# gynvael/MythTracer

Measured on AMD Instinct MI355X. Metric: Mray/s (primary+shadow+secondary; ray = one OctTree::IntersectRay), higher is better.
Workload: dtype f64

## Files before the change

### include/mythtracer_hip.h

```cpp
#ifndef MYTHTRACER_HIP_H_
#define MYTHTRACER_HIP_H_

#include <stdint.h>

#ifdef __cplusplus
extern "C" {
#endif

#define MT_ABI_VERSION 5

enum {
  MT_OK = 0,
  MT_ERR_ARG = -1,
  MT_ERR_HIP = -2,
  MT_ERR_UNSUPPORTED = -3,
  MT_ERR_NOMEM = -4,
  MT_ERR_INTERNAL = -5
};

#define MT_MAX_TREE_DEPTH 64
#define MT_MAX_RECURSION 16

typedef struct mt_material {
  double ambient[3], diffuse[3], specular[3];
// ... 301 lines not shown
  MT_TUNE_HYBRID_QUAD_SHARE,
  MT_TUNE_HYBRID_WORK1, MT_TUNE_HYBRID_WORK2,
  MT_TUNE_FORECAST_STEP,
  MT_TUNE_HYBRID_STARTER_SHARE,
  MT_TUNE_DEEP_LAYOUT,
  MT_TUNE_MULTI_FORCE_PEER_COPY,
  MT_TUNE_MULTI_BALANCE,
  MT_TUNE_XCD_QUEUES,
  MT_TUNE_ORDER_GROUPS,
  MT_TUNE_SM_CELL_SHARE,
  MT_TUNE_SM_CELL_TIME, MT_TUNE_SM_CELL_WORK,
  MT_TUNE_HYBRID_CELL_FACTOR,
  MT_TUNE_LEAN_KERNEL,
  MT_TUNE_COUNT
};
int mt_scene_set_tuning(mt_scene *scene, int knob, double value);

int mt_scene_kernel_times(mt_scene *scene, int max_n, double *primary_ms,
                          double *render_ms);

typedef struct mt_lean_info {
  int32_t lean, handed_over;
  uint32_t units, redo_units;
  double lean_ms, redo_ms;
} mt_lean_info;
int mt_scene_lean_info(mt_scene *scene, mt_lean_info *out);

int mt_intersect_rays(mt_scene *scene, int n, const double *rays,
                      int32_t *tri, int32_t *line_no, double *t,
                      double *point, mt_stats *stats);
// ... 58 lines not shown
```

### mythtracer_amd/binding.py

```python
from __future__ import annotations

import ctypes as C
import os
import weakref

import numpy as np

PKG = os.path.dirname(os.path.abspath(__file__))
HIP_LIB = os.path.join(PKG, "lib", "libmythtracer_hip.so")
HOST_LIB = os.path.join(PKG, "lib", "libmythtracer_host.so")

MT_OK = 0
MT_ABI_VERSION = 5
MT_TEX_RGB8, MT_TEX_F64 = 0, 1

HIP_SYMBOLS = [
    "mt_last_error", "mt_abi_version", "mt_device_count", "mt_scene_create",
    "mt_scene_destroy", "mt_scene_set_lights", "mt_render_chunk",
    "mt_render_chunk_device", "mt_render_tiles_device", "mt_blit_tiles_device",
    "mt_scene_read_stats", "mt_intersect_rays", "mt_scene_set_traversal_mode",
    "mt_scene_kernel_times", "mt_scene_lean_info", "mt_scene_set_scheduling", "mt_scene_set_engine",
    "mt_scene_set_stats", "mt_set_default_engine", "mt_scene_set_tuning",
    "mt_render_frame_multi", "mt_scene_export_costs_device", "mt_scene_import_costs_device",
    "mt_order_tiles_device", "mt_dealt_tile_count", "mt_deal_tiles_device",
# ... 17 lines not shown
    "mt_scene_set_triangle_normals", "mt_scene_set_triangle_uvw", "mt_scene_get_triangle_normals",
    "mt_scene_get_triangle_uvw", "mt_raytree_attr_info_last",
    "mt_octree_build", "mt_octree_info", "mt_octree_read", "mt_octree_destroy", "mt_scene_create_triangles",
    "mt_scene_read_tree",
    "mt_scene_set_triangle_vertices", "mt_scene_get_triangle_vertices", "mt_scene_move_times_last",
]
MT_MAX_RECURSION = 16

TUNE = {name: i for i, name in enumerate([
    "POOL_BELOW", "POOL_CAP", "PACKED_STACK", "BLOCKS_PER_CU", "FORECAST_RADIUS", "BLEND", "FORMS",
    "POOL_CUT_SHARE", "POOL_PIECE_TIME1", "POOL_PIECE_TIME2", "POOL_PIECE_WORK1", "POOL_PIECE_WORK2",
    "POOL_CELL_FACTOR", "QUAD_SHARE", "QUAD_SHARE_MOVING", "QUAD_KEEP", "QUAD_WORK", "QUAD_WORK_MOVING",
    "POOL_SCRATCH_MB", "HYBRID_POOL_SHARE", "HYBRID_QUAD_SHARE", "HYBRID_WORK1", "HYBRID_WORK2", "FORECAST_STEP",
    "HYBRID_STARTER_SHARE", "DEEP_LAYOUT", "MULTI_FORCE_PEER_COPY", "MULTI_BALANCE", "XCD_QUEUES",
    "ORDER_GROUPS", "SM_CELL_SHARE", "SM_CELL_TIME", "SM_CELL_WORK", "HYBRID_CELL_FACTOR", "LEAN_KERNEL"])}

STAT_NAMES = ["rays_primary", "rays_secondary", "rays_shadow", "box_tests",
              "node_visits", "tri_tests", "mt_tests", "shaded_hits"]


class NativeLibraryMissing(RuntimeError):
    pass


class mt_material(C.Structure):
    _fields_ = [("ambient", C.c_double * 3), ("diffuse", C.c_double * 3),
                ("specular", C.c_double * 3), ("specular_exp", C.c_double),
                ("reflectance", C.c_double), ("transparency", C.c_double),
                ("transmission_filter", C.c_double * 3),
                ("refraction_index", C.c_double), ("tex", C.c_int32),
# ... 991 lines not shown
    def read_stats(self, h) -> dict:
        st = mt_stats()
        self.check(self.lib.mt_scene_read_stats(h, C.byref(st)))
        return st.as_dict()

    def set_stats(self, h, enabled: bool):
        self.check(self.lib.mt_scene_set_stats(h, 1 if enabled else 0))

    def set_engine(self, h, engine: int):
        self.check(self.lib.mt_scene_set_engine(h, int(engine)))

    def set_default_engine(self, engine: int):
        self.check(self.lib.mt_set_default_engine(int(engine)))

    def set_tuning(self, h, knob: str, value: float):
        self.check(self.lib.mt_scene_set_tuning(h, TUNE[knob], float(value)))

    def render_frame_multi(self, handles, sensor12, image_w, image_h, tile_w=64, tile_h=64, max_depth=5,
                           want_stats=True):
        n = len(handles)
        arr = (C.c_void_p * n)(*handles)
        rgb = np.zeros((image_h, image_w, 3), dtype=np.uint8)
        st = (mt_stats * n)()
        s = self.make_sensor(sensor12)
        self.check(self.lib.mt_render_frame_multi(C.cast(arr, C.c_void_p), n, C.byref(s), image_w, image_h,
                                                  tile_w, tile_h, max_depth, _ptr(rgb),
                                                  C.cast(st, C.c_void_p) if want_stats else None))
        return dict(rgb=rgb, stats=[st[i].as_dict() for i in range(n)])

    def export_costs_device(self, h, d_map, map_w, map_h, stream=None):
        self.check(self.lib.mt_scene_export_costs_device(h, d_map, map_w, map_h, stream))
# ... 635 lines not shown
```

### mythtracer_amd/csrc/mt_capi.hip

```cpp
#include <hip/hip_runtime.h>
#include <algorithm>
#include <atomic>
#include <map>
#include <memory>
#include <mutex>
#include <string>
#include <thread>
#include <limits>
#include <utility>

#include <chrono>
#include <cmath>
#include <cstdarg>
#include <cstddef>
#include <cstdio>
#include <cstdlib>
#include <cstring>
#include <unistd.h>
#include <vector>

#include "mt_render.hip"
#include "mt_resolve.h"
#include "mt_adaptive.h"
#include "mt_gbuffer.h"
// ... 196 lines not shown
struct mt_scene {
  int device = 0;
  DevScene dev{};
  DeviceAllocs geo, tables;
  TriArrays tri;
  mt_material *mtls = nullptr;
  DevTexture *texs = nullptr;
  Buf<mt_light> d_lights;
  Buf<unsigned long long> d_counters;
  Buf<unsigned int> d_work;
  Buf<unsigned int> d_queues;
  Buf<unsigned int> d_order_ctl;
  Buf<unsigned int> d_order_whist;
  unsigned order_epoch = 0;
  DevScene dev_uploaded;
  bool dev_uploaded_valid = false;
  Buf<double> d_frames;
  Buf<int32_t> d_hit_prim;
  Buf<double> d_hit_t;
  Buf<unsigned int> d_class_list;
  Buf<char> d_pool;
  int engine = 0;
  ForecastBank bank0;
  std::unique_ptr<ForecastBank> bank1;
  void forget_histories() {
    bank0.cost_signature = 0;
    if (bank1) bank1->cost_signature = 0;
    lean_fresh = true;
  }
  bool lean_fresh = true;
// ... 833 lines not shown
  MT_TRY(geo.upload(L.supers, "the super boxes", &dev->sup_aabb32));
  MT_TRY(geo.upload(L.subs, "the subtree boxes", &dev->sub_aabb32));
  MT_TRY(geo.upload(L.hsr, "the walk's records", &dev->hs_rec));
  MT_TRY(geo.upload(L.ll_tri, "the long lists", &dev->ll_tri));
  MT_TRY(geo.upload(L.ll_exact, "the long lists", &dev->ll_exact));
  MT_TRY(geo.upload(L.ll_box_q, "the long lists' boxes", &dev->ll_box_q));
  MT_TRY(geo.upload(L.ll_grp_q, "the long lists' boxes", &dev->ll_grp_q));
  MT_TRY(geo.upload(L.ll_sup_q, "the long lists' boxes", &dev->ll_sup_q));
  MT_TRY(geo.upload(L.sl_box, "the short lists' boxes", &dev->sl_box32));
  MT_TRY(geo.upload(L.recs, "the node records", &dev->nodes));
  MT_TRY(geo.upload(L.tri_aabb, "the triangles' boxes", &dev->tri_aabb));
  MT_TRY(geo.upload(L.tri_aabb32, "the triangles' boxes", &dev->tri_aabb32));
  for (int k = 0; k < 3; k++) dev->bmax[k] = L.bmax[k];
  dev->tree_depth = L.max_depth;
  dev->scene_regular = L.regular ? 1 : 0;
  return MT_OK;
}

static void show_tri_arrays(const TriArrays &tri, DevScene *dev) {
  dev->tri_vertex = tri.vertex;
  dev->tri_normal = tri.normal;
  dev->tri_uvw = tri.uvw;
  dev->tri_mtl = tri.mtl;
  dev->tri_line = tri.line;
}

static int upload_layout(mt_scene *s, const mt_scene_desc *d, const SceneLayout &L) {
  HIP_TRY(hipSetDevice(d->device));
  s->device = d->device;
  hipDeviceProp_t prop;
// ... 23 lines not shown
    texs[i] = DevTexture{dev_texels, t.width, t.height, t.format, 0};
  }
  MT_TRY(s->tables.upload(d->materials, (size_t)d->n_materials, "the materials", &s->mtls));
  s->dev.mtls = s->mtls;
  s->n_materials = d->n_materials;
  s->n_textures = d->n_textures;
  if (d->n_materials > 0) s->mtls_host.assign(d->materials, d->materials + d->n_materials);
  MT_TRY(s->tables.upload(texs, "the texture table", &s->texs));
  s->dev.texs = s->texs;
  s->texs_host = texs;
  s->tex_generation.assign(texs.size(), 0ull);
  s->dev.n_tris = d->n_tris;
  s->dev.n_nodes = d->n_nodes;
  s->dev.force_mode = 0;
  s->dev.pack_shift = pack_shift_for(d->n_tris, d->n_nodes);
  s->dev.n_lights = 0;
  s->dev.lights = nullptr;
  return MT_OK;
}

static int init_launch_state(mt_scene *s) {
  MT_TRY(s->d_counters.ensure(ST_COUNT * sizeof(unsigned long long)));
  HIP_TRY(hipMemset(s->d_counters, 0, ST_COUNT * sizeof(unsigned long long)));
  MT_TRY(s->d_work.ensure((kLeanCtl + 8) * sizeof(unsigned)));
  HIP_TRY(hipMemset(s->d_work, 0, (kLeanCtl + 8) * sizeof(unsigned)));
  MT_TRY(s->d_queues.ensure(kQueueWords * sizeof(unsigned)));
  MT_TRY(s->d_order_ctl.ensure(kOrdWords * sizeof(unsigned)));
  HIP_TRY(hipMemset(s->d_order_ctl, 0, kOrdWords * sizeof(unsigned)));
  MT_TRY(s->d_order_whist.ensure((size_t)kOrdGroupsMax * kOrdKeysMax * sizeof(unsigned)));
  HIP_TRY(hipEventCreate(&s->ev0));
// ... 280 lines not shown

int mt_scene_set_engine(mt_scene *s, int engine) {
  if (!s || engine < 0 || engine > 3) return fail(MT_ERR_ARG, "engine must be 0 (automatic), 1, 2 or 3");
  s->engine = engine;
  s->forget_histories();
  return MT_OK;
}

int mt_set_default_engine(int engine) {
  if (engine < 0 || engine > 3) return fail(MT_ERR_ARG, "engine must be 0 (automatic), 1, 2 or 3");
  g_default_engine.store(engine);
  return MT_OK;
}

int mt_scene_set_tuning(mt_scene *s, int knob, double value) {
  if (!s || knob < 0 || knob >= MT_TUNE_COUNT || !std::isfinite(value)) return fail(MT_ERR_ARG, "bad tuning argument");
  switch (knob) {
    case MT_TUNE_POOL_PIECE_TIME1: case MT_TUNE_POOL_PIECE_TIME2: case MT_TUNE_POOL_PIECE_WORK1: case MT_TUNE_POOL_PIECE_WORK2:
    case MT_TUNE_POOL_CELL_FACTOR: case MT_TUNE_QUAD_SHARE: case MT_TUNE_QUAD_SHARE_MOVING: case MT_TUNE_QUAD_KEEP:
    case MT_TUNE_QUAD_WORK: case MT_TUNE_QUAD_WORK_MOVING: case MT_TUNE_HYBRID_POOL_SHARE: case MT_TUNE_HYBRID_QUAD_SHARE:
    case MT_TUNE_SM_CELL_SHARE: case MT_TUNE_SM_CELL_TIME: case MT_TUNE_SM_CELL_WORK: case MT_TUNE_HYBRID_CELL_FACTOR:
    case MT_TUNE_HYBRID_WORK1: case MT_TUNE_HYBRID_WORK2: case MT_TUNE_FORECAST_STEP: case MT_TUNE_HYBRID_STARTER_SHARE:
      if (!(value >= 1e-6 && value <= 1e6)) return fail(MT_ERR_ARG, "tuning knob %d must lie in [1e-6, 1e6]", knob);
      break;
    case MT_TUNE_POOL_BELOW: case MT_TUNE_POOL_CAP: case MT_TUNE_BLOCKS_PER_CU:
      if (!(value >= 0.0 && value <= 1e9)) return fail(MT_ERR_ARG, "tuning knob %d must lie in [0, 1e9]", knob);
      break;
    case MT_TUNE_POOL_SCRATCH_MB:
      if (!(value >= 1.0 && value <= 1e9)) return fail(MT_ERR_ARG, "the ray pool's scratch budget must lie in [1, 1e9] MB");
      break;
// ... 2937 lines not shown
```

### mythtracer_amd/csrc/mt_device.h

```cpp
#pragma once
#include <hip/hip_runtime.h>
#include <stddef.h>
#include <stdint.h>
#include "mythtracer_hip.h"

#ifndef MT_WAVES_PER_SIMD
#define MT_WAVES_PER_SIMD 2
#endif

namespace mt {

struct NodeRec {
  double lo[3];
  double c[3];
  double hi[3];
  int32_t first_child;
  int32_t prim_begin;
  int32_t prim_count;
  int32_t child_mask;
  int32_t level;
  int32_t pad1;
};
static_assert(sizeof(NodeRec) == 96, "NodeRec must be 96 bytes");

// ... 59 lines not shown
  const double *tri_vertex;
  const double *tri_normal;
  const double *tri_uvw;
  const int32_t *tri_mtl;
  const int32_t *tri_line;
  const mt_material *mtls;
  const DevTexture *texs;
  const mt_light *lights;
  int32_t n_lights;
  int32_t n_tris;
  int32_t n_nodes;
  int32_t tree_depth;
  int32_t force_mode;
  int32_t scene_regular;
  int32_t pack_shift;
  volatile unsigned long long *hb;
  unsigned long long *prof;
  char *deep_base;
  unsigned long long deep_stride;
  const DevScene *self;
};

constexpr int kProfTimeline = 16384;
enum { PROF_TRACE = 0, PROF_SCAN_RAYPAR, PROF_SCAN_TRANSPOSED, PROF_CHILDREN_UNWIND, PROF_N_RAYPAR,
       PROF_N_TRANSPOSED, PROF_N_CHUNKS, PROF_N_RAYPAR_TRIS, PROF_N_TRACES, PROF_SHADE,
       PROF_SCAN_M2F, PROF_SCAN_M2, PROF_SCAN_M1, PROF_SCAN_M0, PROF_N_M2F, PROF_N_M2, PROF_N_M1, PROF_N_M0,
       PROF_TRIS_M2F, PROF_TRIS_M1, PROF_TRIS_TRANSPOSED,
       PROF_G_GROUPS, PROF_G_LIVE, PROF_G_RANGES, PROF_G_RANGE_TRIS,
       PROF_NIN_SUM, PROF_NIN_LT8, PROF_NIN_LT24, PROF_WANT_SUM,
       PROF_TA_G, PROF_TB_G, PROF_TA_T, PROF_TB_T, PROF_TC_T, PROF_T_RAYS, PROF_M2F_CALL,
// ... 122 lines not shown
```

### mythtracer_amd/csrc/mt_layout.h

```cpp
#pragma once
#include <algorithm>
#include <cmath>
#include <cstdarg>
#include <cstddef>
#include <cstdio>
#include <cstring>
#include <string>
#include <utility>
#include <vector>

#include "mt_device.h"

namespace mt {

struct LayoutError {
  int code = MT_OK;
  std::string msg;
};

inline bool refuse(LayoutError *err, int code, const char *fmt, ...) {
  char text[1024];
  va_list ap;
  va_start(ap, fmt);
  vsnprintf(text, sizeof text, fmt, ap);
  va_end(ap);
  err->code = code;
// ... 79 lines not shown

struct SceneLayout {
  std::vector<NodeRec> recs;
  std::vector<float> groups;
  std::vector<float> supers;
  std::vector<float> subs;
  std::vector<HsRec> hsr;
  std::vector<float> sl_box;
  std::vector<int32_t> ll_tri;
  std::vector<double> ll_exact;
  std::vector<float> ll_box_q, ll_grp_q, ll_sup_q;
  std::vector<double> tri_aabb;
  std::vector<float> tri_aabb32;
  double bmax[3] = {0.0, 0.0, 0.0};
  bool regular = false;
  int max_depth = 0;
};


constexpr double kInvertedBox[6] = {3.0e38, 3.0e38, 3.0e38, -3.0e38, -3.0e38, -3.0e38};
static_assert((float)3.0e38 == 3.0e38f, "the fp32 inverted box is the rounded fp64 one");

template <typename T>
inline void box_invert(T *u) {
  for (int k = 0; k < 6; k++) u[k] = (T)kInvertedBox[k];
}

template <typename T>
inline void box_union(T *u, const T *b, size_t n = 1) {
  for (size_t j = 0; j < n; j++, b += 6) {
// ... 253 lines not shown
}

inline void derive_layout(const mt_scene_desc &d, const std::vector<int> &depth_of, SceneLayout *out) {
  SceneLayout &L = *out;
  L = SceneLayout();
  L.regular = scene_regular(d);
  L.max_depth = *std::max_element(depth_of.begin(), depth_of.end());
  derive_node_records(d, depth_of, &L.recs);
  derive_block_boxes(d, &L.groups, &L.supers);
  derive_subtree_boxes(d, &L.recs, &L.subs);
  derive_hit_set_records(d, L.recs, L.subs, &L.hsr, &L.sl_box);
  std::vector<float> ll_box;
  derive_long_lists(d, &L.hsr, &L.ll_tri, &L.ll_exact, &ll_box);
  derive_long_list_quads(ll_box, &L);
  derive_triangle_boxes(d, &L);
}

}
```

### mythtracer_amd/csrc/mt_render.hip

```cpp
#include "mt_shade.h"
#include "mt_pool.h"

namespace mt {

enum { MODE_RADIANCE = 0, MODE_SHADOW = 1 };
enum { STAGE_REFL = 0, STAGE_REFR = 1 };

constexpr int kParkSlots = 18;
enum { PARK_START = 0, PARK_LP = 3, PARK_ADD1 = 6, PARK_ADD2 = 9, PARK_ADD3 = 12, PARK_DIR = 15 };
struct FrameIO {
  double *base;
  double *park;
  int lane;
  __device__ __forceinline__ void park3(int s, V3 v) const {
    park[(s + 0) * 64 + lane] = v.x; park[(s + 1) * 64 + lane] = v.y; park[(s + 2) * 64 + lane] = v.z;
  }
  __device__ __forceinline__ V3 unpark3(int s) const {
    return V3{park[(s + 0) * 64 + lane], park[(s + 1) * 64 + lane], park[(s + 2) * 64 + lane]};
  }
  __device__ __forceinline__ double *slot(int level, int s) const {
    return base + ((size_t)level * kFrameSlots + s) * 64 + lane;
  }
  __device__ __forceinline__ void put3(int level, int s, V3 v) const {
    *slot(level, s) = v.x; *slot(level, s + 1) = v.y; *slot(level, s + 2) = v.z;
// ... 330 lines not shown
    }

    const unsigned long long item_t0 = __builtin_amdgcn_s_memtime();
#ifdef MT_DIAG
    unsigned long long diag_trace_ticks = 0;
#endif
    const ItemGeom g = item_geometry<!LEAN>(P, item, sub, lane);
    bool alive = g.inside;
    const size_t px_index = g.px_index;

    const bool quad = sub >= 0;
    const int R = quad ? 4 : 1;
    const int role = quad ? (lane & 3) : 0;
    const bool owner = role == 0;
    const unsigned long long my_group = quad ? (0xFull << (lane & ~3)) : (1ull << lane);
    enum { MODE_IDLE = 2 };
    int mode = owner ? MODE_RADIANCE : MODE_IDLE;
    int level = 0;
    bool in_object = false;
    double coef = 1.0;
    V3 ro = cam_origin, rd = v3(0, 0, 1);
    if (alive) {
      const V3 d = s_start + (s_ds * (double)g.py) + (s_dp * (double)g.px);
      rd = normalized(d);
    }
    V3 Pt = v3(0, 0, 0), Nn = Pt, surf = Pt, color = Pt;
    bool has_light = false, has_add3 = false, crossed = false;
    double refl_dot = 0.0;
    int mtl = -1, li = 0, round_base = 0;
    bool traversing = false;
    bool want_round = false, waiting_round = false;

    const long long pass_bound =
        (2ll << P.max_depth) * (1 + (long long)S.n_lights * ((long long)S.n_tris + 2)) + 16;
    long long passes = 0;
    while (__ballot(alive) != 0ull) {
      int prim = -1;
      double t = 0.0;
      if (heartbeat) {
        const unsigned long long am = __ballot(alive);
        const unsigned long long ex = __builtin_amdgcn_read_exec();
        if (lane == 0) {
          S.hb[wave_id * 4 + 0] = 2 | ((unsigned long long)passes << 8);
          S.hb[wave_id * 4 + 2] = am;
          S.hb[wave_id * 4 + 3] = ex;
        }
      }
      int trc = DEV_OK;
      const bool tracing = alive && mode != MODE_IDLE;
      if (passes == 0 && from_primary) {
        prim = tracing ? P.hit_prim[px_index] : -1;
        t = tracing ? P.hit_t[px_index] : 0.0;
      } else {
#ifdef MT_DIAG
        const unsigned long long diag_tt0 = __builtin_amdgcn_s_memtime();
#endif
        const TraceOut to = trace_wave<STATS, DEEP, LEAN>(S.self, stk.base, lane, tracing, ro.x, ro.y, ro.z, rd.x, rd.y, rd.z);
#ifdef MT_DIAG
        asm volatile("" :: "v"(to.prim));
        diag_trace_ticks += __builtin_amdgcn_s_memtime() - diag_tt0;
#endif
        add_trace_stats<STATS>(st, to);
        prim = to.prim;
        t = to.t;
        trc = to.status;
        if (LEAN && __builtin_amdgcn_readfirstlane(trc) == DEV_NEEDS_FULL) {
          abandon = true;
          break;
        }
      }
      if (heartbeat) {
        const unsigned long long ex = __builtin_amdgcn_read_exec();
        if (lane == 0) { S.hb[wave_id * 4 + 0] = 3 | ((unsigned long long)passes << 8); S.hb[wave_id * 4 + 3] = ex; }
      }
      if (trc != DEV_OK || ++passes > pass_bound) {
        if (lane == 0) atomicMax(P.counters + ST_STATUS, (unsigned long long)(trc != DEV_OK ? trc : DEV_ERR_PIXEL_BOUND));
        alive = false;
        break;
      }

      bool after_lights = false, do_return = false;
      V3 retval = v3(0, 0, 0);
      V3 add1 = retval, add2 = retval, add3 = retval;
      if (tracing) {
        if (mode == MODE_RADIANCE) {
          if (STATS) {
            if (level > 0) st.v[ST_RAYS_SECONDARY]++;
            else if (!from_primary) st.v[ST_RAYS_PRIMARY]++;
          }
          if (prim < 0) {
            do_return = true;
          } else {
            if (STATS) {
              st.v[ST_SHADED_HITS]++;
              st.v[ST_BYTES_VECTOR] += 72u + 72u + 4u + 64u;
            }
            Pt = ro + rd * t;
            const V3 dir = rd;
            const double *vtx = S.tri_vertex + (size_t)prim * 9;
// ... 16 lines not shown
              if (m->tex >= 0) {
                const V3 uvw = interpolate(S.tri_uvw + (size_t)prim * 9, w);
                surf = surf * texture_color_at(S.texs[m->tex], uvw.x, uvw.y);
              }
              const V3 Rd = dir - Nn * (2 * dot(dir, Nn));
              refl_dot = dot(Rd, towards_camera);
              fio.park3(PARK_DIR, dir);
              color = v3(0, 0, 0);
              round_base = 0;
              if (S.n_lights > 0) want_round = true;
              else after_lights = true;
              mode = MODE_IDLE;
            }
          }
        } else {
          if (STATS) {
            st.v[ST_RAYS_SHADOW]++;
            st.v[ST_BYTES_VECTOR] += 96u + 4u + 32u;
          }
          const MT_CONST mt_light *lt = lights + li;
          const V3 lpos = v3(lt->position[0], lt->position[1], lt->position[2]);
          bool light_done = false, in_shadow = false;
          V3 start = Pt, lp = v3(1.0, 1.0, 1.0);
          if (crossed) {
            start = fio.unpark3(PARK_START);
            lp = fio.unpark3(PARK_LP);
          }
          if (prim < 0) {
            light_done = true;
          } else {
// ... 48 lines not shown
              const V3 ls = v3(lt->specular[0], lt->specular[1], lt->specular[2]);
              add3 = ks * surf * ::pow(refl_dot, m->specular_exp) * ls;
              has_add3 = true;
            }
            if (quad) {
              fio.park3(PARK_ADD1, add1);
              fio.park3(PARK_ADD2, add2);
              fio.park3(PARK_ADD3, add3);
            }
            mode = MODE_IDLE;
          }
        }
      }

      {
        const unsigned long long busy = __ballot(alive && mode == MODE_SHADOW);
        const bool round_done = owner && waiting_round && ((busy & my_group) == 0ull);
        const int hl0 = has_light ? 1 : 0, h30 = has_add3 ? 1 : 0;
        if (quad && has_light) {
          add1 = fio.unpark3(PARK_ADD1);
          add2 = fio.unpark3(PARK_ADD2);
          add3 = fio.unpark3(PARK_ADD3);
        }
        if (round_done && has_light) {
          color = color + add1;
          color = color + add2;
          if (has_add3) color = color + add3;
        }
        if (quad) {
          const int hl1 = quad_get_i32<1>(hl0), hl2 = quad_get_i32<2>(hl0), hl3 = quad_get_i32<3>(hl0);
          const int h31 = quad_get_i32<1>(h30), h32 = quad_get_i32<2>(h30), h33 = quad_get_i32<3>(h30);
// ... 275 lines not shown
```

### mythtracer_amd/csrc/mt_trace.h

```cpp
#pragma once
#include <type_traits>
#include "mt_device.h"

namespace mt {

#define MT_CONST __attribute__((address_space(4)))
#define MT_CNT_ADD(i, v) (cntr[i] += (v))
#define MT_CNT_SET(i, v) (cntr[i] = (v))
#define MT_CNT_GET(i) (cntr[i])

#ifndef MT_PACK_SMALL
#define MT_PACK_SMALL 8
#endif

#ifdef MT_PROF
#define MT_PROF_DECL unsigned long long prof_acc[PROF_COUNT] = {0}; unsigned long long prof_t0 = 0, prof_t1 = 0
#define MT_PROF_BEGIN(var) var = __builtin_amdgcn_s_memtime()
#define MT_PROF_END(slot, var) prof_acc[slot] += __builtin_amdgcn_s_memtime() - var
#define MT_PROF_COUNT(slot, n) prof_acc[slot] += (unsigned long long)(n)
#define MT_TL(tag) do { if (tl_on && tl_i < 512u && tl_base + tl_i < (unsigned long long)kProfTimeline) { \
    S.prof[PROF_COUNT + 1 + tl_base + tl_i] = (__builtin_amdgcn_s_memtime() << 8) | (unsigned)(tag); tl_i++; } } while (0)
#define MT_PROF_FLUSH(ptr, lane) do { if ((ptr) && (lane) == 0) { for (int pi_ = 0; pi_ < PROF_COUNT; pi_++) if (prof_acc[pi_]) atomicAdd((ptr) + pi_, prof_acc[pi_]); } } while (0)
#else
#define MT_PROF_DECL
// ... 195 lines not shown

struct RayRegs {
  double ox, oy, oz;
  double dx, dy, dz;
  double ix, iy, iz;
};
#define MT_RAY_PARAMS double ox_, double oy_, double oz_, double dx_, double dy_, double dz_, \
                      double ix_, double iy_, double iz_
#define MT_RAY_ARGS(r) (r).ox, (r).oy, (r).oz, (r).dx, (r).dy, (r).dz, (r).ix, (r).iy, (r).iz
#define MT_F32_PARAMS float fix_, float fiy_, float fiz_, float fcnx_, float fcny_, float fcnz_, \
                      float fcfx_, float fcfy_, float fcfz_
#define MT_F32_ARGS(f) (f).ix, (f).iy, (f).iz, (f).cnx, (f).cny, (f).cnz, (f).cfx, (f).cfy, (f).cfz
#define MT_F32_FROM_PARAMS(f) \
  Filter32 f;                 \
  f.ix = fix_; f.iy = fiy_; f.iz = fiz_; f.cnx = fcnx_; f.cny = fcny_; f.cnz = fcnz_; \
  f.cfx = fcfx_; f.cfy = fcfy_; f.cfz = fcfz_
#define MT_RAY_FROM_PARAMS(r) \
  RayRegs r;                  \
  r.ox = ox_; r.oy = oy_; r.oz = oz_; r.dx = dx_; r.dy = dy_; r.dz = dz_; r.ix = ix_; r.iy = iy_; r.iz = iz_

template <bool STATS>
__device__ __forceinline__ void flush_candidates(const DevScene &S, const RayRegs &r,
                                                 int &pend, int &best, double &best_t,
                                                 LaneStats &st) {
  if (pend >= 0) {
    double t;
    if (STATS) {
      st.v[ST_MT_TESTS]++;
      st.v[ST_BYTES_VECTOR] += 72u;
    }
    if (moller_trumbore(S.tri_vertex + (size_t)pend * 9, r.ox, r.oy, r.oz, r.dx, r.dy, r.dz, &t)) {
// ... 98 lines not shown
    if (k >= pc) break;
    p += 24;
    issue_pair(A, p);
    scan_pair<MODE, OCT, STATS>(S, r, B, pb, k, pc, pend, pmask, best, best_t, st);
    await_pair(A);
    k += 2;
    if (k >= pc) break;
  }
  if (pmask) flush_candidates<STATS>(S, r, pend, best, best_t, st);
}

struct Filter32 {
  float ix, iy, iz;
  float cnx, cny, cnz;
  float cfx, cfy, cfz;
};

__device__ __forceinline__ float f32_pred(float f) {
  unsigned b = __builtin_bit_cast(unsigned, f);
  if ((b & 0x7fffffffu) == 0u) return __builtin_bit_cast(float, 0x80000001u);
  b = (b & 0x80000000u) ? b + 1u : b - 1u;
  return __builtin_bit_cast(float, b);
}
__device__ __forceinline__ float f32_succ(float f) {
  unsigned b = __builtin_bit_cast(unsigned, f);
  if ((b & 0x7fffffffu) == 0u) return __builtin_bit_cast(float, 0x00000001u);
  b = (b & 0x80000000u) ? b - 1u : b + 1u;
  return __builtin_bit_cast(float, b);
}
__device__ __forceinline__ float f32_not_above(double c) {
// ... 80 lines not shown
  const float b0 = b[0], b1 = b[1], b2 = b[2], b3 = b[3], b4 = b[4], b5 = b[5];
  const float tnx = __builtin_fmaf(sx ? b3 : b0, f.ix, f.cnx), tfx = __builtin_fmaf(sx ? b0 : b3, f.ix, f.cfx);
  const float tny = __builtin_fmaf(sy ? b4 : b1, f.iy, f.cny), tfy = __builtin_fmaf(sy ? b1 : b4, f.iy, f.cfy);
  const float tnz = __builtin_fmaf(sz ? b5 : b2, f.iz, f.cnz), tfz = __builtin_fmaf(sz ? b2 : b5, f.iz, f.cfz);
  const float lo = __builtin_fmaxf(__builtin_fmaxf(tnx, tny), tnz);
  const float hi = __builtin_fminf(__builtin_fminf(tfx, tfy), tfz);
  return !(hi < 0.0f) && !(lo > hi);
}

__device__ __forceinline__ bool near_far_may_hit(float nx, float fx, float ny, float fy, float nz, float fz, const Filter32 &f) {
  const float tnx = __builtin_fmaf(nx, f.ix, f.cnx), tfx = __builtin_fmaf(fx, f.ix, f.cfx);
  const float tny = __builtin_fmaf(ny, f.iy, f.cny), tfy = __builtin_fmaf(fy, f.iy, f.cfy);
  const float tnz = __builtin_fmaf(nz, f.iz, f.cnz), tfz = __builtin_fmaf(fz, f.iz, f.cfz);
  const float lo0 = __builtin_fmaxf(__builtin_fmaxf(tnx, tny), __builtin_fmaxf(tnz, 0.0f));
  const float hi = __builtin_fminf(__builtin_fminf(tfx, tfy), tfz);
  return !(lo0 > hi);
}

__device__ __forceinline__ unsigned degenerate_children(const DevScene *self, const float *sub, int fc, double ox,
                                                        double oy, double oz, double ix, double iy, double iz) {
  const int axis = degenerate_axis(ox, oy, oz, ix, iy, iz);
  if (axis < 0) return 0xffu;
  const double o = axis == 0 ? ox : (axis == 1 ? oy : oz);
  (void)self;
  (void)fc;
  return degenerate_keep_mask(sub, axis, o);
}

typedef float f16v __attribute__((ext_vector_type(16)));
typedef float f8v __attribute__((ext_vector_type(8)));
// ... 1008 lines not shown

struct TraceOut {
  int status;
  int prim;
  double t;
  unsigned box_tests, node_visits, tri_tests, mt_tests, bytes_vector;
  unsigned wave_node_steps, wave_tri_steps, bytes_scalar;

};

#ifdef MT_TRACE_CALL
#define MT_TRACE_ATTR __attribute__((noinline))
#else
#define MT_TRACE_ATTR __forceinline__
#endif
template <bool STATS, int DEEP = 0, bool LEAN = false>
__device__ MT_TRACE_ATTR TraceOut trace_wave(const DevScene *scene, unsigned stack_base, int lane,
                                                         bool want_all, double ox, double oy, double oz,
                                                         double dx, double dy, double dz) {
  constexpr bool WIDE = DEEP >= 2;
  const MT_CONST DevScene *G = as_const(uniform_ptr(scene));
  DevScene S;
  S.nodes = G->nodes;
  S.tri_aabb = G->tri_aabb;
  S.tri_aabb32 = G->tri_aabb32;
  S.grp_aabb32 = G->grp_aabb32;
  S.sub_aabb32 = G->sub_aabb32;
  S.hs_rec = G->hs_rec;
  S.sl_box32 = G->sl_box32;
  S.ll_box_q = G->ll_box_q;
  S.ll_grp_q = G->ll_grp_q;
  S.ll_sup_q = G->ll_sup_q;
  S.ll_tri = G->ll_tri;
  S.ll_exact = G->ll_exact;
// ... 56 lines not shown
  out_prim = -1;
  out_t = 0.0;

  const bool fin = __builtin_isfinite(ox) && __builtin_isfinite(oy) && __builtin_isfinite(oz) &&
                   __builtin_isfinite(r.ix) && __builtin_isfinite(r.iy) && __builtin_isfinite(r.iz) &&
                   r.ix != 0.0 && r.iy != 0.0 && r.iz != 0.0;
  const int rounds = (!LEAN && S.scene_regular != 0 && S.force_mode != 1 && __ballot(want_all && !fin) != 0ull &&
                      __ballot(want_all && fin) != 0ull) ? 2 : 1;
  int status = DEV_OK;
  for (int round = 0; round < rounds; round++) {
  const bool want = rounds == 1 ? want_all : (want_all && (fin == (round == 0)));
  const bool all_regular = (S.scene_regular != 0) && (S.force_mode != 1) &&
                           (__ballot(want && !fin) == 0ull);
  Filter32 f32;
  const bool f32_ok = make_filter32(S, r, f32);
  const bool use_filter = all_regular && (S.force_mode != 4) && (S.force_mode != 2) &&
                          (__ballot(want && !f32_ok) == 0ull);

  const bool cull = use_filter && (S.force_mode != 7);
  const bool irr_boxes = !all_regular && (S.scene_regular != 0) && (S.force_mode == 0) &&
                         S.bmax[0] <= 0x1p400 && S.bmax[1] <= 0x1p400 && S.bmax[2] <= 0x1p400;

  const MT_CONST NodeRec *nodes = as_const(S.nodes);
  int cur = -1;
  if (want) {
    const MT_CONST NodeRec *R = nodes;
    if (STATS) {
      MT_CNT_SET(0, 1u);
      st.bytes_scalar += 96u;
    }
// ... 351 lines not shown
      }
      {
        const double t0 = (P->lo[1] - r.oy) * r.iy, tc = (P->c[1] - r.oy) * r.iy, t1 = (P->hi[1] - r.oy) * r.iy;
        amax[1][0] = mx<false>(t0, tc); amin[1][0] = mn<false>(t0, tc);
        amax[1][1] = mx<false>(tc, t1); amin[1][1] = mn<false>(tc, t1);
      }
      {
        const double t0 = (P->lo[2] - r.oz) * r.iz, tc = (P->c[2] - r.oz) * r.iz, t1 = (P->hi[2] - r.oz) * r.iz;
        amax[2][0] = mx<false>(t0, tc); amin[2][0] = mn<false>(t0, tc);
        amax[2][1] = mx<false>(tc, t1); amin[2][1] = mn<false>(tc, t1);
      }
      const bool xh = (slot_ & 1) != 0, zh = (slot_ & 2) != 0, yh = (slot_ & 4) != 0;
      const double tmax = mn3<false>(xh ? amax[0][1] : amax[0][0], yh ? amax[1][1] : amax[1][0], zh ? amax[2][1] : amax[2][0]);
      const double tmin = mx3<false>(xh ? amin[0][1] : amin[0][0], yh ? amin[1][1] : amin[1][0], zh ? amin[2][1] : amin[2][0]);
      const bool entered = (tmax >= 0.0) & (tmin <= tmax);
      const int own_p = HS_LD(h_own_p, g_own_p, lev);
      const double own_t = HS_LD(h_own_t, g_own_t, lev);
      if (rp_ >= 0 && entered && !(own_p >= 0 && rt_ > own_t)) {
        const int wp = HS_LD(h_win_p, g_win_p, lev);
        bool take = wp < 0;
        if (!take) {
          const int kw = (int)((unsigned)wp >> 28);
          const bool wxh = (kw & 1) != 0, wzh = (kw & 2) != 0, wyh = (kw & 4) != 0;
          const double wmin = mx3<false>(wxh ? amin[0][1] : amin[0][0], wyh ? amin[1][1] : amin[1][0], wzh ? amin[2][1] : amin[2][0]);
          take = (tmin < wmin) || (tmin == wmin && slot_ < kw);
        }
        if (take) {
          HS_ST(h_win_p, g_win_p, lev, rp_ | (slot_ << 28));
          HS_ST(h_win_t, g_win_t, lev, rt_);
        }
      }
      {
        unsigned rest = get8(pendA, pendB, pendC, lev);
        if (rest != 0u) {
          const int wp = HS_LD(h_win_p, g_win_p, lev);
          const int kw = (int)((unsigned)wp >> 28) & 7;
          const bool wxh = (kw & 1) != 0, wzh = (kw & 2) != 0, wyh = (kw & 4) != 0;
          const double wmin = mx3<false>(wxh ? amin[0][1] : amin[0][0], wyh ? amin[1][1] : amin[1][0], wzh ? amin[2][1] : amin[2][0]);
          unsigned my = get8(wantA, wantB, wantC, lev);
          unsigned still = 0u;
          while (rest != 0u) {
            const int c2 = __builtin_ctz(rest);
            rest &= rest - 1u;
            const bool cxh = (c2 & 1) != 0, czh = (c2 & 2) != 0, cyh = (c2 & 4) != 0;
            const double cmin = mx3<false>(cxh ? amin[0][1] : amin[0][0], cyh ? amin[1][1] : amin[1][0], czh ? amin[2][1] : amin[2][0]);
            const bool behind = wp >= 0 && !((cmin < wmin) || (cmin == wmin && c2 < kw));
            if (behind) my &= ~(1u << c2);
            if (__ballot(((my >> c2) & 1u) != 0u) != 0ull) still |= 1u << c2;
          }
          set8(wantA, wantB, wantC, lev, my);
          set8(pendA, pendB, pendC, lev, still);
        }
      }
    };
    if (m != 0ull) {
      hs_fetch(0);
      for (;;) {
      if (++steps > step_bound) {
        status = DEV_ERR_TRAVERSAL_BOUND;
        break;
      }
      lev = uniform_i32(lev);
      node = uniform_i32(node);
      slot = uniform_i32(slot);
      entering = uniform_i32(entering ? 1 : 0) != 0;
      pendA = uniform_u64(pendA);
      pendB = uniform_u64(pendB);
// ... 47 lines not shown
          const MT_LDS f4v *ky = (const MT_LDS f4v *)(uintptr_t)(rec + 112u + (syl != 0 ? 32u : 0u));
          const MT_LDS f4v *kz = (const MT_LDS f4v *)(uintptr_t)(rec + 208u + (szl != 0 ? 32u : 0u));
          float pnx[8], pfx[8], pny[8], pfy[8], pnz[8], pfz[8];
#pragma unroll
          for (int i = 0; i < 2; i++) {
            const f4v a = kx[i], b = kx[2 + i], c = ky[i], d = ky[2 + i], e = kz[i], g = kz[2 + i];
            pnx[i * 4 + 0] = a.x; pnx[i * 4 + 1] = a.y; pnx[i * 4 + 2] = a.z; pnx[i * 4 + 3] = a.w;
            pfx[i * 4 + 0] = b.x; pfx[i * 4 + 1] = b.y; pfx[i * 4 + 2] = b.z; pfx[i * 4 + 3] = b.w;
            pny[i * 4 + 0] = c.x; pny[i * 4 + 1] = c.y; pny[i * 4 + 2] = c.z; pny[i * 4 + 3] = c.w;
            pfy[i * 4 + 0] = d.x; pfy[i * 4 + 1] = d.y; pfy[i * 4 + 2] = d.z; pfy[i * 4 + 3] = d.w;
            pnz[i * 4 + 0] = e.x; pnz[i * 4 + 1] = e.y; pnz[i * 4 + 2] = e.z; pnz[i * 4 + 3] = e.w;
            pfz[i * 4 + 0] = g.x; pfz[i * 4 + 1] = g.y; pfz[i * 4 + 2] = g.z; pfz[i * 4 + 3] = g.w;
          }
#pragma unroll
          for (int c = 0; c < 8; c++) {
            const bool pass = near_far_may_hit(pnx[c], pfx[c], pny[c], pfy[c], pnz[c], pfz[c], f32);
            if (pass) bits |= 1u << c;
            if ((__ballot(pass) & m) != 0ull) any |= 1u << c;
          }
          bits = in ? (bits & cm) : 0u;
          any &= cm;
        }
        MT_TL(4);
        bool in_list = false;
        if (pc > 0) {
          const MT_LDS float *wx = (const MT_LDS float *)(uintptr_t)(rec + (unsigned)kHsRecOwn + (sxl != 0 ? 4u : 0u));
          const MT_LDS float *wy = (const MT_LDS float *)(uintptr_t)(rec + (unsigned)kHsRecOwn + 12u + (syl != 0 ? 4u : 0u));
          const MT_LDS float *wz = (const MT_LDS float *)(uintptr_t)(rec + (unsigned)kHsRecOwn + 24u + (szl != 0 ? 4u : 0u));
          in_list = in && near_far_may_hit(wx[0], wx[1], wy[0], wy[1], wz[0], wz[1], f32);
        }
        const unsigned long long lm = __ballot(in_list);
#ifdef MT_PROF
        asm volatile("" :: "v"(bits), "s"(any), "s"(lm));
        MT_PROF_END(PROF_HS_KIDS_T, prof_t1);
        MT_PROF_BEGIN(prof_t1);
#endif
        MT_TL(5);
        int best = -1;
        double best_t = 0.0;
        if (small_list && lm != 0ull) {
          wait_vm(0);
          unsigned long long cand = in_list ? list_bits(tstage, pc) : 0ull;
          if (STATS) st.bytes_scalar += 24u * (unsigned)pc;
          unsigned mt = 0u, bv = 0u;
// ... 79 lines not shown
          slot = lev >= 0 ? closed - __builtin_amdgcn_readlane(lane_fc, lev) : 0;
          continue;
        }
        MT_TL(9);
        const int c = pick(todo);
        set8(pendA, pendB, pendC, lev, todo & ~(1u << c));
        m = __ballot(((get8(wantA, wantB, wantC, lev) >> c) & 1u) != 0u);
        node = __builtin_amdgcn_readlane(lane_fc, lev) + c;
        entering = true;
      }
      }
    }
    if (want && status == DEV_OK) {
      out_prim = ret_p;
      out_t = ret_t;
    }
    cur = -1;
  }
  if constexpr (!LEAN)
  if (!hs_done)
  {
  for (;;) {
    if (lane_phase) {
      MT_PROF_BEGIN(prof_t1);
#if MT_PACK_SMALL > 0
      if (!all_regular) {
        for (int guard = 0;; guard++) {
          const bool mine = cur >= 0 && cur_pc < kBigNode;
          const unsigned long long need = __ballot(mine);
          if (need == 0ull || __builtin_popcountll(need) > MT_PACK_SMALL) break;
// ... 260 lines not shown
```

Baseline: 2494.

## Bound shadow-ray traversal by conservative light distance to prune far nodes

Adds a host-computed conservative error bound (rho1, mu, kappa) for regular octrees and passes each shadow ray's light distance into trace_wave. The f32 box filter then clips node and list tests at a float tmax, so subtrees beyond the light are skipped. Exact ties are flagged and re-traced unbounded through a new MODE_SHADOW_AGAIN state. This adds a per-scene validation pass, a redo path, extra registers in the traversal kernel and a looser pass bound. By default it is only enabled for launches without stats counters (knob 1).

```diff
diff --git a/include/mythtracer_hip.h b/include/mythtracer_hip.h
--- a/include/mythtracer_hip.h
+++ b/include/mythtracer_hip.h
@@ -339,6 +339,7 @@
   MT_TUNE_LEAN_KERNEL,
   MT_TUNE_COUNT
 };
+#define MT_TUNE_SHADOW_BOUND 1000
 int mt_scene_set_tuning(mt_scene *scene, int knob, double value);
 
 int mt_scene_kernel_times(mt_scene *scene, int max_n, double *primary_ms,
diff --git a/mythtracer_amd/binding.py b/mythtracer_amd/binding.py
--- a/mythtracer_amd/binding.py
+++ b/mythtracer_amd/binding.py
@@ -55,6 +55,7 @@
     "POOL_SCRATCH_MB", "HYBRID_POOL_SHARE", "HYBRID_QUAD_SHARE", "HYBRID_WORK1", "HYBRID_WORK2", "FORECAST_STEP",
     "HYBRID_STARTER_SHARE", "DEEP_LAYOUT", "MULTI_FORCE_PEER_COPY", "MULTI_BALANCE", "XCD_QUEUES",
     "ORDER_GROUPS", "SM_CELL_SHARE", "SM_CELL_TIME", "SM_CELL_WORK", "HYBRID_CELL_FACTOR", "LEAN_KERNEL"])}
+TUNE_EXTRA = {"SHADOW_BOUND": 1000}
 
 STAT_NAMES = ["rays_primary", "rays_secondary", "rays_shadow", "box_tests",
               "node_visits", "tri_tests", "mt_tests", "shaded_hits"]
@@ -1076,7 +1077,7 @@
         self.check(self.lib.mt_set_default_engine(int(engine)))
 
     def set_tuning(self, h, knob: str, value: float):
-        self.check(self.lib.mt_scene_set_tuning(h, TUNE[knob], float(value)))
+        self.check(self.lib.mt_scene_set_tuning(h, TUNE[knob] if knob in TUNE else TUNE_EXTRA[knob], float(value)))
 
     def render_frame_multi(self, handles, sensor12, image_w, image_h, tile_w=64, tile_h=64, max_depth=5,
                            want_stats=True):
diff --git a/mythtracer_amd/csrc/mt_capi.hip b/mythtracer_amd/csrc/mt_capi.hip
--- a/mythtracer_amd/csrc/mt_capi.hip
+++ b/mythtracer_amd/csrc/mt_capi.hip
@@ -234,6 +234,7 @@
   Buf<unsigned int> d_order_whist;
   unsigned order_epoch = 0;
   DevScene dev_uploaded;
+  int32_t shadow_bound_knob = 1;
   bool dev_uploaded_valid = false;
   Buf<double> d_frames;
   Buf<int32_t> d_hit_prim;
@@ -1097,6 +1098,7 @@
   for (int k = 0; k < 3; k++) dev->bmax[k] = L.bmax[k];
   dev->tree_depth = L.max_depth;
   dev->scene_regular = L.regular ? 1 : 0;
+  dev->sb = L.shadow;
   return MT_OK;
 }
 
@@ -1150,6 +1152,7 @@
   s->dev.n_nodes = d->n_nodes;
   s->dev.force_mode = 0;
   s->dev.pack_shift = pack_shift_for(d->n_tris, d->n_nodes);
+  s->dev.sb_knob = s->shadow_bound_knob;
   s->dev.n_lights = 0;
   s->dev.lights = nullptr;
   return MT_OK;
@@ -1460,6 +1463,12 @@
 }
 
 int mt_scene_set_tuning(mt_scene *s, int knob, double value) {
+  if (s && knob == MT_TUNE_SHADOW_BOUND) {
+    if (!(value == 0.0 || value == 1.0 || value == 2.0)) return fail(MT_ERR_ARG, "shadow bound: 0 (never), 1 (launches without work counters) or 2 (always)");
+    s->shadow_bound_knob = s->dev.sb_knob = (int32_t)value;
+    s->forget_histories();
+    return MT_OK;
+  }
   if (!s || knob < 0 || knob >= MT_TUNE_COUNT || !std::isfinite(value)) return fail(MT_ERR_ARG, "bad tuning argument");
   switch (knob) {
     case MT_TUNE_POOL_PIECE_TIME1: case MT_TUNE_POOL_PIECE_TIME2: case MT_TUNE_POOL_PIECE_WORK1: case MT_TUNE_POOL_PIECE_WORK2:
diff --git a/mythtracer_amd/csrc/mt_device.h b/mythtracer_amd/csrc/mt_device.h
--- a/mythtracer_amd/csrc/mt_device.h
+++ b/mythtracer_amd/csrc/mt_device.h
@@ -3,6 +3,7 @@
 #include <stddef.h>
 #include <stdint.h>
 #include "mythtracer_hip.h"
+#include "mt_shadow_bound.h"
 
 #ifndef MT_WAVES_PER_SIMD
 #define MT_WAVES_PER_SIMD 2
@@ -97,6 +98,8 @@
   int32_t force_mode;
   int32_t scene_regular;
   int32_t pack_shift;
+  ShadowBound sb;
+  int32_t sb_knob;
   volatile unsigned long long *hb;
   unsigned long long *prof;
   char *deep_base;
diff --git a/mythtracer_amd/csrc/mt_layout.h b/mythtracer_amd/csrc/mt_layout.h
--- a/mythtracer_amd/csrc/mt_layout.h
+++ b/mythtracer_amd/csrc/mt_layout.h
@@ -10,6 +10,7 @@
 #include <vector>
 
 #include "mt_device.h"
+#include "mt_shadow_bound.h"
 
 namespace mt {
 
@@ -119,6 +120,7 @@
   std::vector<float> tri_aabb32;
   double bmax[3] = {0.0, 0.0, 0.0};
   bool regular = false;
+  ShadowBound shadow{1.0f, 0.0f, 0.0f, 0};
   int max_depth = 0;
 };
 
@@ -402,6 +404,11 @@
   derive_long_lists(d, &L.hsr, &L.ll_tri, &L.ll_exact, &ll_box);
   derive_long_list_quads(ll_box, &L);
   derive_triangle_boxes(d, &L);
-}
-
-}
+  if (L.regular) {
+    const ShadowBoundInput in{d.n_nodes, d.n_tris, d.node_aabb, d.node_center, d.node_first_child, d.node_prim_begin,
+                              d.node_prim_count, d.tri_vertex, d.tri_aabb};
+    L.shadow = shadow_bound_for(in);
+  }
+}
+
+}
diff --git a/mythtracer_amd/csrc/mt_render.hip b/mythtracer_amd/csrc/mt_render.hip
--- a/mythtracer_amd/csrc/mt_render.hip
+++ b/mythtracer_amd/csrc/mt_render.hip
@@ -368,7 +368,7 @@
     const int role = quad ? (lane & 3) : 0;
     const bool owner = role == 0;
     const unsigned long long my_group = quad ? (0xFull << (lane & ~3)) : (1ull << lane);
-    enum { MODE_IDLE = 2 };
+    enum { MODE_IDLE = 2, MODE_SHADOW_AGAIN = 3 };
     int mode = owner ? MODE_RADIANCE : MODE_IDLE;
     int level = 0;
     bool in_object = false;
@@ -386,7 +386,7 @@
     bool want_round = false, waiting_round = false;
 
     const long long pass_bound =
-        (2ll << P.max_depth) * (1 + (long long)S.n_lights * ((long long)S.n_tris + 2)) + 16;
+        (2ll << P.max_depth) * (1 + 2 * (long long)S.n_lights * ((long long)S.n_tris + 2)) + 16;
     long long passes = 0;
     while (__ballot(alive) != 0ull) {
       int prim = -1;
@@ -409,7 +409,12 @@
 #ifdef MT_DIAG
         const unsigned long long diag_tt0 = __builtin_amdgcn_s_memtime();
 #endif
-        const TraceOut to = trace_wave<STATS, DEEP, LEAN>(S.self, stk.base, lane, tracing, ro.x, ro.y, ro.z, rd.x, rd.y, rd.z);
+        float l32 = __builtin_inff();
+        if (tracing && mode == MODE_SHADOW) {
+          const MT_CONST mt_light *lt = lights + li;
+          l32 = shadow_l32(sqr_distance(ro, v3(lt->position[0], lt->position[1], lt->position[2])));
+        }
+        const TraceOut to = trace_wave<STATS, DEEP, LEAN, true>(S.self, stk.base, lane, tracing, ro.x, ro.y, ro.z, rd.x, rd.y, rd.z, l32);
 #ifdef MT_DIAG
         asm volatile("" :: "v"(to.prim));
         diag_trace_ticks += __builtin_amdgcn_s_memtime() - diag_tt0;
@@ -436,7 +441,9 @@
       bool after_lights = false, do_return = false;
       V3 retval = v3(0, 0, 0);
       V3 add1 = retval, add2 = retval, add3 = retval;
-      if (tracing) {
+      const bool again = tracing && prim == kTraceRedo;
+      if (again) mode = MODE_SHADOW_AGAIN;
+      if (tracing && !again) {
         if (mode == MODE_RADIANCE) {
           if (STATS) {
             if (level > 0) st.v[ST_RAYS_SECONDARY]++;
@@ -483,6 +490,7 @@
             }
           }
         } else {
+          mode = MODE_SHADOW;
           if (STATS) {
             st.v[ST_RAYS_SHADOW]++;
             st.v[ST_BYTES_VECTOR] += 96u + 4u + 32u;
@@ -561,7 +569,7 @@
       }
 
       {
-        const unsigned long long busy = __ballot(alive && mode == MODE_SHADOW);
+        const unsigned long long busy = __ballot(alive && (mode & 1) != 0);
         const bool round_done = owner && waiting_round && ((busy & my_group) == 0ull);
         const int hl0 = has_light ? 1 : 0, h30 = has_add3 ? 1 : 0;
         if (quad && has_light) {
diff --git a/mythtracer_amd/csrc/mt_shadow_bound.h b/mythtracer_amd/csrc/mt_shadow_bound.h
--- /dev/null
+++ b/mythtracer_amd/csrc/mt_shadow_bound.h
@@ -0,0 +1,140 @@
+#pragma once
+#include <cmath>
+#include <cstdint>
+#include <cstring>
+
+#if defined(__HIPCC__) || defined(__CUDACC__)
+#define MT_SB_HD __host__ __device__
+#else
+#define MT_SB_HD
+#endif
+
+namespace mt {
+
+struct ShadowBound {
+  float rho1;
+  float mu;
+  float kappa;
+  int32_t on;
+};
+
+MT_SB_HD inline float sb_f32_not_below(double c) {
+  float f = (float)c;
+  if ((double)f < c) {
+    uint32_t b;
+    memcpy(&b, &f, 4);
+    if ((b & 0x7fffffffu) == 0u) b = 0x00000001u;
+    else b = (b & 0x80000000u) ? b - 1u : b + 1u;
+    memcpy(&f, &b, 4);
+  }
+  return f;
+}
+
+MT_SB_HD inline float shadow_l32(double dist2) { return sqrtf(sb_f32_not_below(dist2)); }
+MT_SB_HD inline float shadow_tmax32(const ShadowBound &b, float l32, float imax) {
+  return (l32 * b.rho1 + b.mu) + b.kappa * imax;
+}
+
+struct ShadowBoundInput {
+  int n_nodes, n_tris;
+  const double *node_aabb, *node_center;
+  const int32_t *node_first_child, *node_prim_begin, *node_prim_count;
+  const double *tri_vertex, *tri_aabb;
+};
+
+constexpr double kSbTau = 0.00000001;
+constexpr double kSbMaxCoord = 0x1p40;
+
+struct ShadowSlop {
+  double a, r, dt, diag;
+};
+inline ShadowSlop shadow_slop(double longest_edge, const double *root_box) {
+  ShadowSlop s;
+  double d2 = 0.0;
+  for (int k = 0; k < 3; k++) d2 += (root_box[3 + k] - root_box[k]) * (root_box[3 + k] - root_box[k]);
+  s.diag = std::sqrt(d2) * (1.0 + 0x1p-30);
+  s.dt = s.diag + 1e-3;
+  s.a = 12.0 * 0x1p-53 * longest_edge * longest_edge / kSbTau;
+  s.r = 4.0 * s.a * (s.dt + 2.0 * longest_edge);
+  return s;
+}
+
+inline void sb_octant(const double *lo, const double *c, const double *hi, int k, double *out) {
+  const bool high[3] = {(k & 1) != 0, (k & 4) != 0, (k & 2) != 0};
+  for (int a = 0; a < 3; a++) {
+    out[a] = high[a] ? c[a] : lo[a];
+    out[3 + a] = high[a] ? hi[a] : c[a];
+  }
+}
+
+inline ShadowBound shadow_bound_for(const ShadowBoundInput &d, const char **why = nullptr) {
+  ShadowBound off{1.0f, 0.0f, 0.0f, 0};
+  const char *dummy;
+  if (!why) why = &dummy;
+  *why = "";
+  auto no = [&](const char *w) { *why = w; return off; };
+  if (d.n_nodes < 1 || d.n_tris < 1) return no("no triangles");
+  auto sane = [](const double *p, size_t n) {
+    for (size_t i = 0; i < n; i++) {
+      if (!(std::fabs(p[i]) <= kSbMaxCoord)) return false;
+    }
+    return true;
+  };
+  if (!sane(d.node_aabb, (size_t)d.n_nodes * 6) || !sane(d.node_center, (size_t)d.n_nodes * 3) ||
+      !sane(d.tri_aabb, (size_t)d.n_tris * 6) || !sane(d.tri_vertex, (size_t)d.n_tris * 9)) {
+    return no("a coordinate is not finite or beyond 2^40");
+  }
+  double e2max = 0.0;
+  for (int t = 0; t < d.n_tris; t++) {
+    const double *v = d.tri_vertex + (size_t)t * 9, *b = d.tri_aabb + (size_t)t * 6;
+    for (int a = 0; a < 3; a++) {
+      if (!(b[a] <= b[3 + a])) return no("a triangle's box is inverted");
+      for (int j = 0; j < 3; j++) {
+        if (!(b[a] <= v[j * 3 + a] && v[j * 3 + a] <= b[3 + a])) return no("a triangle's vertex lies outside its box");
+      }
+    }
+    for (int j = 0; j < 3; j++) {
+      const double *p = v + j * 3, *q = v + ((j + 1) % 3) * 3;
+      const double l2 = (p[0] - q[0]) * (p[0] - q[0]) + (p[1] - q[1]) * (p[1] - q[1]) + (p[2] - q[2]) * (p[2] - q[2]);
+      if (l2 > e2max) e2max = l2;
+    }
+  }
+  for (int i = 0; i < d.n_nodes; i++) {
+    const double *bx = d.node_aabb + (size_t)i * 6, *c = d.node_center + (size_t)i * 3;
+    for (int a = 0; a < 3; a++) {
+      if (!(bx[a] <= bx[3 + a])) return no("a node's box is inverted");
+    }
+    const int pb = d.node_prim_begin[i], pc = d.node_prim_count[i];
+    for (int t = pb; t < pb + pc; t++) {
+      const double *b = d.tri_aabb + (size_t)t * 6;
+      for (int a = 0; a < 3; a++) {
+        if (!(bx[a] <= b[a] && b[3 + a] <= bx[3 + a])) return no("a triangle's box pokes out of its node's cell");
+      }
+    }
+    const int fc = d.node_first_child[i];
+    if (fc == 0) continue;
+    for (int a = 0; a < 3; a++) {
+      if (!(bx[a] <= c[a] && c[a] <= bx[3 + a])) return no("a node's centre lies outside its box");
+    }
+    for (int k = 0; k < 8; k++) {
+      double o[6];
+      sb_octant(bx, c, bx + 3, k, o);
+      if (memcmp(o, d.node_aabb + (size_t)(fc + k) * 6, sizeof o) != 0) return no("a child's box is not its octant");
+    }
+  }
+  const ShadowSlop s = shadow_slop(std::sqrt(e2max) * (1.0 + 0x1p-30), d.node_aabb);
+  if (!(s.a <= 1.0 / 64.0)) return no("the longest edge makes the arithmetic's slop too large");
+  const double rho = 6.0 * s.a / (1.0 - 6.0 * s.a);
+  const double m32 = 1.0 + 0x1p-18;
+  const double mu = (3.0 * s.a * s.dt * (1.0 + rho) + 2e-5 * (1.0 + rho)) * m32;
+  const double kappa = 3.0 * s.r * (1.0 + rho) * m32;
+  if (!std::isfinite(mu) || !std::isfinite(kappa) || !(mu <= s.diag)) return no("mu exceeds the scene's diagonal");
+  ShadowBound b;
+  b.rho1 = sb_f32_not_below((1.0 + rho) * m32);
+  b.mu = sb_f32_not_below(mu);
+  b.kappa = sb_f32_not_below(kappa);
+  b.on = 1;
+  return b;
+}
+
+}
diff --git a/mythtracer_amd/csrc/mt_trace.h b/mythtracer_amd/csrc/mt_trace.h
--- a/mythtracer_amd/csrc/mt_trace.h
+++ b/mythtracer_amd/csrc/mt_trace.h
@@ -233,7 +233,7 @@
 #define MT_F32_FROM_PARAMS(f) \
   Filter32 f;                 \
   f.ix = fix_; f.iy = fiy_; f.iz = fiz_; f.cnx = fcnx_; f.cny = fcny_; f.cnz = fcnz_; \
-  f.cfx = fcfx_; f.cfy = fcfy_; f.cfz = fcfz_
+  f.cfx = fcfx_; f.cfy = fcfy_; f.cfz = fcfz_; f.tmax = __builtin_inff()
 #define MT_RAY_FROM_PARAMS(r) \
   RayRegs r;                  \
   r.ox = ox_; r.oy = oy_; r.oz = oz_; r.dx = dx_; r.dy = dy_; r.dz = dz_; r.ix = ix_; r.iy = iy_; r.iz = iz_
@@ -362,6 +362,7 @@
   float ix, iy, iz;
   float cnx, cny, cnz;
   float cfx, cfy, cfz;
+  float tmax;
 };
 
 __device__ __forceinline__ float f32_pred(float f) {
@@ -472,6 +473,14 @@
   const float tnz = __builtin_fmaf(nz, f.iz, f.cnz), tfz = __builtin_fmaf(fz, f.iz, f.cfz);
   const float lo0 = __builtin_fmaxf(__builtin_fmaxf(tnx, tny), __builtin_fmaxf(tnz, 0.0f));
   const float hi = __builtin_fminf(__builtin_fminf(tfx, tfy), tfz);
+  return !(lo0 > hi);
+}
+__device__ __forceinline__ bool near_far_may_hit_within(float nx, float fx, float ny, float fy, float nz, float fz, const Filter32 &f) {
+  const float tnx = __builtin_fmaf(nx, f.ix, f.cnx), tfx = __builtin_fmaf(fx, f.ix, f.cfx);
+  const float tny = __builtin_fmaf(ny, f.iy, f.cny), tfy = __builtin_fmaf(fy, f.iy, f.cfy);
+  const float tnz = __builtin_fmaf(nz, f.iz, f.cnz), tfz = __builtin_fmaf(fz, f.iz, f.cfz);
+  const float lo0 = __builtin_fmaxf(__builtin_fmaxf(tnx, tny), __builtin_fmaxf(tnz, 0.0f));
+  const float hi = __builtin_fminf(__builtin_fminf(__builtin_fminf(tfx, tfy), tfz), f.tmax);
   return !(lo0 > hi);
 }
 
@@ -1510,10 +1519,11 @@
 #else
 #define MT_TRACE_ATTR __forceinline__
 #endif
-template <bool STATS, int DEEP = 0, bool LEAN = false>
+constexpr int kTraceRedo = -2;
+template <bool STATS, int DEEP = 0, bool LEAN = false, bool BOUNDED = false>
 __device__ MT_TRACE_ATTR TraceOut trace_wave(const DevScene *scene, unsigned stack_base, int lane,
                                                          bool want_all, double ox, double oy, double oz,
-                                                         double dx, double dy, double dz) {
+                                                         double dx, double dy, double dz, float l32 = __builtin_inff()) {
   constexpr bool WIDE = DEEP >= 2;
   const MT_CONST DevScene *G = as_const(uniform_ptr(scene));
   DevScene S;
@@ -1600,6 +1610,14 @@
                            (__ballot(want && !fin) == 0ull);
   Filter32 f32;
   const bool f32_ok = make_filter32(S, r, f32);
+  f32.tmax = __builtin_inff();
+  if constexpr (BOUNDED) {
+    ShadowBound sb;
+    sb.rho1 = G->sb.rho1; sb.mu = G->sb.mu; sb.kappa = G->sb.kappa;
+    const bool sb_on = G->sb.on != 0 && G->sb_knob > (STATS ? 1 : 0);
+    const float imax = __builtin_fmaxf(__builtin_fmaxf(__builtin_fabsf(f32.ix), __builtin_fabsf(f32.iy)), __builtin_fabsf(f32.iz));
+    if (sb_on) f32.tmax = shadow_tmax32(sb, l32, imax);
+  }
   const bool use_filter = all_regular && (S.force_mode != 4) && (S.force_mode != 2) &&
                           (__ballot(want && !f32_ok) == 0ull);
 
@@ -1981,6 +1999,8 @@
       const double tmax = mn3<false>(xh ? amax[0][1] : amax[0][0], yh ? amax[1][1] : amax[1][0], zh ? amax[2][1] : amax[2][0]);
       const double tmin = mx3<false>(xh ? amin[0][1] : amin[0][0], yh ? amin[1][1] : amin[1][0], zh ? amin[2][1] : amin[2][0]);
       const bool entered = (tmax >= 0.0) & (tmin <= tmax);
+      const bool bounded_lane = BOUNDED && f32.tmax < __builtin_inff();
+      const bool tie = bounded_lane && rp_ >= 0 && entered && tmin == tmax;
       const int own_p = HS_LD(h_own_p, g_own_p, lev);
       const double own_t = HS_LD(h_own_t, g_own_t, lev);
       if (rp_ >= 0 && entered && !(own_p >= 0 && rt_ > own_t)) {
@@ -2011,13 +2031,16 @@
             rest &= rest - 1u;
             const bool cxh = (c2 & 1) != 0, czh = (c2 & 2) != 0, cyh = (c2 & 4) != 0;
             const double cmin = mx3<false>(cxh ? amin[0][1] : amin[0][0], cyh ? amin[1][1] : amin[1][0], czh ? amin[2][1] : amin[2][0]);
-            const bool behind = wp >= 0 && !((cmin < wmin) || (cmin == wmin && c2 < kw));
+            const bool behind = wp >= 0 && !((cmin < wmin) || (cmin == wmin && (c2 < kw || bounded_lane)));
             if (behind) my &= ~(1u << c2);
             if (__ballot(((my >> c2) & 1u) != 0u) != 0ull) still |= 1u << c2;
           }
           set8(wantA, wantB, wantC, lev, my);
           set8(pendA, pendB, pendC, lev, still);
         }
+      }
+      if constexpr (BOUNDED) {
+        if (tie) f32.tmax = -__builtin_inff();
       }
     };
     if (m != 0ull) {
@@ -2095,7 +2118,8 @@
           }
 #pragma unroll
           for (int c = 0; c < 8; c++) {
-            const bool pass = near_far_may_hit(pnx[c], pfx[c], pny[c], pfy[c], pnz[c], pfz[c], f32);
+            const bool pass = BOUNDED ? near_far_may_hit_within(pnx[c], pfx[c], pny[c], pfy[c], pnz[c], pfz[c], f32)
+                                      : near_far_may_hit(pnx[c], pfx[c], pny[c], pfy[c], pnz[c], pfz[c], f32);
             if (pass) bits |= 1u << c;
             if ((__ballot(pass) & m) != 0ull) any |= 1u << c;
           }
@@ -2108,7 +2132,8 @@
           const MT_LDS float *wx = (const MT_LDS float *)(uintptr_t)(rec + (unsigned)kHsRecOwn + (sxl != 0 ? 4u : 0u));
           const MT_LDS float *wy = (const MT_LDS float *)(uintptr_t)(rec + (unsigned)kHsRecOwn + 12u + (syl != 0 ? 4u : 0u));
           const MT_LDS float *wz = (const MT_LDS float *)(uintptr_t)(rec + (unsigned)kHsRecOwn + 24u + (szl != 0 ? 4u : 0u));
-          in_list = in && near_far_may_hit(wx[0], wx[1], wy[0], wy[1], wz[0], wz[1], f32);
+          in_list = in && (BOUNDED ? near_far_may_hit_within(wx[0], wx[1], wy[0], wy[1], wz[0], wz[1], f32)
+                                   : near_far_may_hit(wx[0], wx[1], wy[0], wy[1], wz[0], wz[1], f32));
         }
         const unsigned long long lm = __ballot(in_list);
 #ifdef MT_PROF
@@ -2218,6 +2243,9 @@
     if (want && status == DEV_OK) {
       out_prim = ret_p;
       out_t = ret_t;
+      if constexpr (BOUNDED) {
+        if (f32.tmax == -__builtin_inff()) out_prim = kTraceRedo;
+      }
     }
     cur = -1;
   }
```

Result: faster. 2715 (median of 6 runs) (+8.9%).
